# NVIDIA/makani

Hardware: NVIDIA H100
Metric: SFNO-block fwd+bwd samples/sec (higher is better)
Workload: dtype tf32

## Files before the change

makani_b200/csrc/dft.cu:

```cuda
#include "umma_common.cuh"
#include "dft_math.cuh"
#include <cmath>
#include <cstdlib>
#include <vector>

namespace b200sht {

int umma_available();

constexpr int kDftMaxHalf = 95;
constexpr int kDftSynWorkers = 10;
constexpr int kDftSynThreads = 32 * (kDftSynWorkers + 2);
constexpr int kDftSynStages = 4;
__host__ __device__ constexpr int dft_out_box(int N2) {
  int d = N2 < 32 ? N2 : 32;
  while (N2 % d != 0) --d;
  return 8 * d;
}

struct DftTables {
  float* et;
  float* eb;
  float2* tw;
  float* zeros;
  int N2, half, M2, nkb;
};

bool dft_shape_ok(int nlon, int mmax) {
  if (nlon % 8 != 0) return false;
  const int N2 = nlon / 8;
  return N2 >= 2 && N2 / 2 <= kDftMaxHalf && (mmax + 7) / 8 <= 32 && mmax <= nlon / 2 + 1;
}

__global__ void dft_tables_kernel(float* et, float* eb, float2* tw, int N2, int half, int M2, int nkb, int nlon) {
  const int i = blockIdx.x * blockDim.x + threadIdx.x;
  if (i < 2 * 128 * 32) {
    const int m2 = i % 32, row = i / 32, p = (row >> 3) & 1, j2 = 8 * (row >> 4) + (row & 7);
    float v = 0.f;
    if (j2 <= half && m2 < M2) {
      const long long t = ((long long)m2 * j2) % N2;
      const double ang = 2.0 * M_PI * (double)t / (double)N2;
      v = tf32_rn((float)(p == 0 ? cos(ang) : sin(ang)));
    }
    et[i] = v;
  }
  if (i < nkb * 2 * 32 * 32) {
    const int jl = i % 32, m2 = (i / 32) % 32, p = (i / 1024) % 2, kb = i / 2048;
    const int j2 = kb * 32 + jl;
    float v = 0.f;
    if (j2 <= half && m2 < M2) {
      const long long t = ((long long)m2 * j2) % N2;
      const double ang = 2.0 * M_PI * (double)t / (double)N2;
      v = tf32_rn((float)(p == 0 ? cos(ang) : sin(ang)));
      if (2 * j2 == N2) v *= 0.5f;
    }
    eb[i] = v;
  }
  if (i < 8 * N2) {
    const int j2 = i % N2, c = i / N2;
    const double ang = 2.0 * M_PI * (double)(c * j2) / (double)nlon;
    tw[i] = make_float2((float)cos(ang), (float)sin(ang));
  }
}

int dft_plan_init(Plan* pl) {
  pl->dft_state = nullptr;
  if (!umma_available()) return -1;
  if (!dft_shape_ok(pl->nlon, pl->mmax)) return -1;
  DftTables* t = new DftTables();
  t->N2 = pl->nlon / 8; t->half = t->N2 / 2; t->M2 = (pl->mmax + 7) / 8;
  t->nkb = (t->half + 1 + 31) / 32;
  t->et = nullptr; t->eb = nullptr; t->tw = nullptr; t->zeros = nullptr;
  const size_t neb = (size_t)t->nkb * 2 * 32 * 32;
  cudaError_t e = cudaMalloc(&t->et, sizeof(float) * 2 * 128 * 32);
  if (e == cudaSuccess) e = cudaMalloc(&t->eb, sizeof(float) * neb);
  if (e == cudaSuccess) e = cudaMalloc(&t->tw, sizeof(float2) * 8 * t->N2);
  if (e == cudaSuccess) e = cudaMalloc(&t->zeros, sizeof(float) * 8 * t->N2);
  if (e == cudaSuccess) e = cudaMemset(t->zeros, 0, sizeof(float) * 8 * t->N2);
  if (e == cudaSuccess) {
    const int n = 8192 > 8 * t->N2 ? 8192 : 8 * t->N2;
    dft_tables_kernel<<<(n + 255) / 256, 256>>>(t->et, t->eb, t->tw, t->N2, t->half, t->M2, t->nkb, pl->nlon);
    e = cudaGetLastError();
    if (e == cudaSuccess) e = cudaStreamSynchronize(0);
  }
  if (e != cudaSuccess) {
    cudaFree(t->et); cudaFree(t->eb); cudaFree(t->tw); cudaFree(t->zeros);
    delete t;
    return -1;
  }
  pl->dft_state = t;
  return 0;
}

void dft_plan_destroy(Plan* pl) {
  DftTables* t = static_cast<DftTables*>(pl->dft_state);
  if (!t) return;
  cudaFree(t->et); cudaFree(t->eb); cudaFree(t->tw); cudaFree(t->zeros);
  delete t;
  pl->dft_state = nullptr;
}

static bool dft_enabled() {
  static const int on = [] { const char* e = getenv("B200SHT_DFT"); return e ? atoi(e) : 1; }();
  return on != 0;
}
bool dft_usable(const Plan* pl) { return pl->dft_state != nullptr && dft_enabled(); }

static unsigned long long* g_dft_prof = nullptr;
static unsigned long long* dft_prof_buffer() {
  static const int on = [] { const char* e = getenv("B200SHT_DFT_PROF"); return e ? atoi(e) : 0; }();
  if (!on) return nullptr;
  if (!g_dft_prof) {
    if (cudaMalloc(&g_dft_prof, 16 * sizeof(unsigned long long)) != cudaSuccess) { g_dft_prof = nullptr; return nullptr; }
    cudaMemset(g_dft_prof, 0, 16 * sizeof(unsigned long long));
  }
  return g_dft_prof;
}
int dft_profile_read(unsigned long long* out16) {
  if (!g_dft_prof) { for (int i = 0; i < 16; ++i) out16[i] = 0; return 0; }
  B200_CHECK_CUDA(cudaDeviceSynchronize());
  B200_CHECK_CUDA(cudaMemcpy(out16, g_dft_prof, 16 * sizeof(unsigned long long), cudaMemcpyDeviceToHost));
  B200_CHECK_CUDA(cudaMemset(g_dft_prof, 0, 16 * sizeof(unsigned long long)));
  return 0;
}
#ifdef B200SHT_DFT_PROFILE
constexpr bool kDftProfile = true;
#else
constexpr bool kDftProfile = false;
#endif
__device__ __forceinline__ void prof_wait(unsigned long long* prof, int slot, uint64_t* bar, uint32_t parity, bool lead) {
  if (!kDftProfile || prof == nullptr) { mbar_wait(bar, parity); return; }
  const long long t0 = clock64();
  mbar_wait(bar, parity);
  if (lead) atomicAdd(prof + slot, (unsigned long long)(clock64() - t0));
}

static int make_tmap_out(CUtensorMap* tm, void* base, bool bf16, int nlon, int nlat, long long rows, int ow) {
  TmapKey key;
  memset(&key, 0, sizeof(key));
  key.base = base; key.rank = 3; key.kind = bf16 ? 7 : 6;
  key.dims[0] = nlon; key.dims[1] = nlat; key.dims[2] = rows; key.box[0] = ow;
  int slot = 0;
  if (tmap_lookup(key, tm, &slot)) return 0;
  PFN_encodeTiled enc = get_encode();
  if (!enc) { set_error("cuTensorMapEncodeTiled is unavailable"); return B200SHT_ERR_UNSUPPORTED; }
  static thread_local bool ctx_bound = false;
  if (!ctx_bound) { cudaFree(nullptr); ctx_bound = true; }
  const int es = bf16 ? 2 : 4;
  cuuint64_t gd[3] = {(cuuint64_t)nlon, (cuuint64_t)nlat, (cuuint64_t)rows};
  cuuint64_t gst[2] = {(cuuint64_t)nlon * es, (cuuint64_t)nlon * nlat * es};
  cuuint32_t bx[3] = {(cuuint32_t)ow, 8, 1}, el[3] = {1, 1, 1};
  if (gst[0] % 16 != 0 || (reinterpret_cast<uintptr_t>(base) & 15) != 0 || (ow * es) % 16 != 0) {
    set_error("tensor map (output): base / row pitch / box row not 16-byte aligned");
    return B200SHT_ERR_INVALID;
  }
  CUresult r = enc(tm, bf16 ? CU_TENSOR_MAP_DATA_TYPE_BFLOAT16 : CU_TENSOR_MAP_DATA_TYPE_FLOAT32, 3, base, gd, gst, bx, el,
                   CU_TENSOR_MAP_INTERLEAVE_NONE, CU_TENSOR_MAP_SWIZZLE_NONE, CU_TENSOR_MAP_L2_PROMOTION_L2_256B, CU_TENSOR_MAP_FLOAT_OOB_FILL_NONE);
  if (r != CUDA_SUCCESS) { set_error("cuTensorMapEncodeTiled (output) failed (%d)", (int)r); return B200SHT_ERR_CUDA; }
  tmap_store(key, tm, slot);
  return 0;
}

template <typename T> __device__ __forceinline__ void st_out(T* p, float v);
template <> __device__ __forceinline__ void st_out<float>(float* p, float v) { *p = v; }
template <> __device__ __forceinline__ void st_out<__nv_bfloat16>(__nv_bfloat16* p, float v) { *p = __float2bfloat16_rn(v); }
template <typename T> __device__ __forceinline__ uint32_t ld_raw(const T* p);
template <> __device__ __forceinline__ uint32_t ld_raw<float>(const float* p) { return __float_as_uint(__ldg(p)); }
template <> __device__ __forceinline__ uint32_t ld_raw<__nv_bfloat16>(const __nv_bfloat16* p) { return (uint32_t)__ldg(reinterpret_cast<const unsigned short*>(p)); }

#ifndef B200_DFT_TF32_MODE
#define B200_DFT_TF32_MODE 2
#endif
constexpr float kTruncComp = 1.0f + 0.0009765625f / 3.0f;
__device__ __forceinline__ float tf32_operand(float v) {
#if B200_DFT_TF32_MODE == 0
  return tf32_rn(v);
#elif B200_DFT_TF32_MODE == 1
  return __uint_as_float((__float_as_uint(v) + 0x1000u) & 0xffffe000u);
#else
  return v;
#endif
}
__device__ __forceinline__ float tf32_operand_unscaled(float v) {
#if B200_DFT_TF32_MODE == 2
  return v * kTruncComp;
#else
  return tf32_operand(v);
#endif
}

__device__ __forceinline__ pr pr_operand(pr v) { return make_pr(tf32_operand(v.v.x), tf32_operand(v.v.y)); }
__device__ __forceinline__ pr pr_operand_unscaled(pr v) {
#if B200_DFT_TF32_MODE == 2
  return rmul(v, kTruncComp);
#else
  return pr_operand(v);
#endif
}

template <typename T> __device__ __forceinline__ float ld_in(const T* p);
template <> __device__ __forceinline__ float ld_in<float>(const float* p) { return __ldg(p); }
template <> __device__ __forceinline__ float ld_in<__nv_bfloat16>(const __nv_bfloat16* p) {
  return __uint_as_float((uint32_t)__ldg(reinterpret_cast<const unsigned short*>(p)) << 16);
}

struct DftSynParams {
  alignas(64) CUtensorMap tmZ;
  alignas(64) CUtensorMap tmE;
  alignas(64) CUtensorMap tmY;
  const float* Z;
  const float2* tw;
  const float* rowscale;
  const float* bias;
  unsigned long long* prof;
  int R, C, nlat, nlon, kp, mmax, N2, half, M2, mode, ntiles, ktiles, has_nyq, ow;
  int kt0, kt_all;
};

template <typename T>
__global__ void __launch_bounds__(kDftSynThreads, 1) dft_synthesis_kernel(const __grid_constant__ DftSynParams p) {
  extern __shared__ uint8_t smem_raw[];
  __shared__ unsigned long long prof_s[16];
  unsigned long long* const prof = (kDftProfile && p.prof) ? prof_s : nullptr;
  if (kDftProfile && threadIdx.x < 16) prof_s[threadIdx.x] = 0;
  const uint32_t raw = smem_u32(smem_raw);
  const uint32_t base = (raw + 1023u) & ~1023u;
  uint8_t* gbase = smem_raw + (base - raw);
  const int N2 = p.N2;
  const int nlon = 8 * N2;
  const int ow = p.ow;
  const uint32_t obytes = (8u * nlon * sizeof(T) + 1023u) & ~1023u;
  const uint32_t sA = base, sB = base + 32768, sO = sB + kDftSynStages * 16384;
  T* const outS = reinterpret_cast<T*>(gbase + (sO - base));
  float2* tws = reinterpret_cast<float2*>(gbase + (sO - base) + 2 * obytes);
  uint64_t* bars = reinterpret_cast<uint64_t*>(reinterpret_cast<uint8_t*>(tws) + ((8 * N2 * 8 + 15) & ~15));
  uint64_t* full = bars;
  uint64_t* empty = full + kDftSynStages;
  uint64_t* e_full = empty + kDftSynStages;
  uint64_t* staged = e_full + 1;
  uint64_t* ofree = staged + 2;

  const int warp = __shfl_sync(0xffffffffu, (int)(threadIdx.x >> 5), 0), lane = threadIdx.x & 31;
  pdl_trigger();
  const int nblk = (p.half + 8) / 8;
  const int nwork = kDftSynWorkers < 2 * nblk ? kDftSynWorkers : 2 * nblk;
  const bool is_tma = (warp == kDftSynWorkers), is_store = (warp == kDftSynWorkers + 1);

  if (threadIdx.x == 0) {
    for (int s = 0; s < kDftSynStages; ++s) { mbar_init(&full[s], 1); mbar_init(&empty[s], nblk); }
    mbar_init(e_full, 1);
    for (int b = 0; b < 2; ++b) { mbar_init(&staged[b], 32 * nblk); mbar_init(&ofree[b], 1); }
    fence_barrier_init();
    prefetch_tmap(&p.tmZ);
    prefetch_tmap(&p.tmE);
    prefetch_tmap(&p.tmY);
  }
  for (int i = threadIdx.x; i < 8 * p.N2; i += blockDim.x) tws[i] = p.tw[i];
  __syncthreads();
  const long long t_cta0 = (kDftProfile && p.prof && threadIdx.x == 0) ? clock64() : 0;
  pdl_wait();

  if (is_tma) {
    if (lane == 0) {
      mbar_expect_tx(e_full, 32768);
      tma_load_2d(sA, &p.tmE, e_full, 0, 0);
      tma_load_2d(sA + 16384, &p.tmE, e_full, 0, 128);
      int n = 0;
      for (int ti = blockIdx.x; ti < p.ntiles; ti += gridDim.x, ++n) {
        const int s = n % kDftSynStages, it = n / kDftSynStages;
        if (it > 0) prof_wait(prof, 8, &empty[s], (it - 1) & 1, true);
        mbar_expect_tx(&full[s], 16384);
        const uint32_t st = sB + s * 16384;
        const int ta = (ti / p.ktiles) * p.kt_all + p.kt0 + ti % p.ktiles;
        tma_load_5d(st, &p.tmZ, &full[s], 0, 0, 0, 0, ta);
        tma_load_5d(st + 4096, &p.tmZ, &full[s], 0, 1, 0, 0, ta);
        tma_load_5d(st + 8192, &p.tmZ, &full[s], 0, 0, 0, 1, ta);
        tma_load_5d(st + 12288, &p.tmZ, &full[s], 0, 1, 0, 1, ta);
      }
    }
    __syncwarp();
  } else if (is_store) {
    if (lane == 0) {
      int n = 0;
      for (int ti = blockIdx.x; ti < p.ntiles; ti += gridDim.x, ++n) {
        const int b = n & 1;
        prof_wait(prof, 11, &staged[b], (n >> 1) & 1, true);
        const int r = ti / p.ktiles, k0 = (p.kt0 + ti - r * p.ktiles) * 8;
// ... 112 lines not shown
      }
    }
  }
  __syncthreads();
  if (kDftProfile && p.prof && threadIdx.x == 0) prof_s[12] = (unsigned long long)(clock64() - t_cta0);
  if (kDftProfile) __syncthreads();
  if (kDftProfile && p.prof && threadIdx.x < 16) atomicAdd(p.prof + threadIdx.x, prof_s[threadIdx.x]);
}

int dft_synthesis(const Plan* pl, const float* Z, void* y, int dtype, int B, int C, const float* bias, int mode, cudaStream_t st, int k_begin, int k_end) {
  const DftTables* t = static_cast<const DftTables*>(pl->dft_state);
  B200_REQUIRE(t != nullptr, "dft_synthesis: plan has no DFT tables");
  const int R = B * C;
  DftSynParams p;
  memset(&p, 0, sizeof(p));
  p.Z = Z; p.tw = t->tw; p.rowscale = pl->d_rowscale; p.bias = bias; p.prof = dft_prof_buffer();
  p.R = R; p.C = C; p.nlat = pl->nlat; p.nlon = pl->nlon; p.kp = pl->kp; p.mmax = pl->mmax;
  p.N2 = t->N2; p.half = t->half; p.mode = mode;
  if (k_end < 0 || k_end > pl->kp) k_end = pl->kp;
  B200_REQUIRE(k_begin >= 0 && k_begin % 8 == 0 && k_begin < k_end, "dft_synthesis: bad latitude range [%d, %d)", k_begin, k_end);
  p.kt_all = pl->kp / 8; p.kt0 = k_begin / 8;
  p.ktiles = (k_end - k_begin + 7) / 8; p.ntiles = R * p.ktiles;
  p.has_nyq = (pl->mmax == pl->nlon / 2 + 1) ? 1 : 0;
  p.M2 = t->M2;
  {
    long long d[5] = {32, 2, t->M2, 2, (long long)R * (pl->kp / 8)}, s[5] = {1, 32, 64, (long long)t->M2 * 64, 2ll * t->M2 * 64};
    int bx[5] = {32, 1, 32, 1, 1};
    int rc = make_tmap(&p.tmZ, Z, 5, d, s, bx);
    if (rc) return rc;
  }
  {
    long long d[2] = {32, 256}, s[2] = {1, 32};
    int bx[2] = {32, 128};
    int rc = make_tmap(&p.tmE, t->et, 2, d, s, bx);
    if (rc) return rc;
  }
  const bool bf16 = (dtype == B200SHT_BF16);
  p.ow = dft_out_box(t->N2);
  {
    int rc = make_tmap_out(&p.tmY, y, bf16, pl->nlon, pl->nlat, R, p.ow);
    if (rc) return rc;
  }
  const size_t obytes = (8 * (size_t)pl->nlon * (bf16 ? 2 : 4) + 1023) & ~(size_t)1023;
  const size_t smem = 1024 + 32768 + (size_t)kDftSynStages * 16384 + 2 * obytes + ((8 * (size_t)t->N2 * 8 + 15) & ~(size_t)15) +
                      (2 * kDftSynStages + 5) * 8;
  const int sms = usable_sms(pl->sm_count > 0 ? pl->sm_count : 132);
  const int ctas = p.ntiles < sms ? p.ntiles : sms;
#define B200_LAUNCH_SYN(TT)                                                                                          \
  do {                                                                                                                \
    struct Tag {};                                                                                                    \
    B200_CHECK_CUDA((ensure_dynamic_smem<Tag>(dft_synthesis_kernel<TT>, smem)));                                     \
    B200_CHECK_CUDA(launch_pdl(dft_synthesis_kernel<TT>, dim3(ctas), dim3(kDftSynThreads), smem, st, p));            \
  } while (0)
  if (bf16) { B200_LAUNCH_SYN(__nv_bfloat16); } else { B200_LAUNCH_SYN(float); }
#undef B200_LAUNCH_SYN
  B200_CHECK_LAUNCH();
  return 0;
}

__host__ __device__ constexpr int dft_box_group(int N2, int es) { return (N2 * es) % 16 == 0 ? 1 : (2 * N2 * es) % 16 == 0 ? 2 : (4 * N2 * es) % 16 == 0 ? 4 : 8; }

static int make_tmap_segments(CUtensorMap* tm, const void* base, bool bf16, int nlon, int gs, long long rows, int box_cols) {
  TmapKey key;
  memset(&key, 0, sizeof(key));
  key.base = base; key.rank = 3; key.kind = bf16 ? 5 : 4;
  key.dims[0] = nlon; key.dims[1] = gs; key.dims[2] = rows; key.box[0] = box_cols;
  int slot = 0;
  if (tmap_lookup(key, tm, &slot)) return 0;
  PFN_encodeTiled enc = get_encode();
  if (!enc) { set_error("cuTensorMapEncodeTiled is unavailable"); return B200SHT_ERR_UNSUPPORTED; }
  static thread_local bool ctx_bound = false;
  if (!ctx_bound) { cudaFree(nullptr); ctx_bound = true; }
  const int es = bf16 ? 2 : 4, N2 = nlon / 8;
  cuuint64_t gd[3] = {(cuuint64_t)gs * N2, (cuuint64_t)(8 / gs), (cuuint64_t)rows};
  cuuint64_t gst[2] = {(cuuint64_t)gs * N2 * es, (cuuint64_t)nlon * es};
  cuuint32_t bx[3] = {(cuuint32_t)box_cols, (cuuint32_t)(8 / gs), 16}, el[3] = {1, 1, 1};
  if (gst[0] % 16 != 0 || gst[1] % 16 != 0 || (reinterpret_cast<uintptr_t>(base) & 15) != 0 || (box_cols * es) % 16 != 0) {
    set_error("tensor map (segments): base / pitch / box row not 16-byte aligned");
    return B200SHT_ERR_INVALID;
  }
  CUresult r = enc(tm, bf16 ? CU_TENSOR_MAP_DATA_TYPE_BFLOAT16 : CU_TENSOR_MAP_DATA_TYPE_FLOAT32, 3, const_cast<void*>(base), gd, gst, bx, el,
                   CU_TENSOR_MAP_INTERLEAVE_NONE, CU_TENSOR_MAP_SWIZZLE_NONE, CU_TENSOR_MAP_L2_PROMOTION_L2_256B, CU_TENSOR_MAP_FLOAT_OOB_FILL_NONE);
  if (r != CUDA_SUCCESS) { set_error("cuTensorMapEncodeTiled (segments) failed (%d)", (int)r); return B200SHT_ERR_CUDA; }
  tmap_store(key, tm, slot);
  return 0;
}

constexpr int kDftAnaStages = 2;
constexpr int kDftAnaMma = 8, kDftAnaLoader = 8, kDftAnaProd0 = 9, kDftAnaThreads = 512;

struct DftAnaParams {
  alignas(64) CUtensorMap tmB;
  alignas(64) CUtensorMap tmXc;
  alignas(64) CUtensorMap tmXp;
  float* X;
  const float2* tw;
  const float* rowscale;
  unsigned long long* prof;
  int R, nlat, nlon, kp, mmax, N2, half, M2, nkb, mode, round_tf32, ntiles, ktiles, nraw, gs;
  int kt0;
};

template <typename T, int N2T>
__global__ void __launch_bounds__(kDftAnaThreads, 1) dft_analysis_kernel(const __grid_constant__ DftAnaParams p) {
  extern __shared__ uint8_t smem_raw[];
  __shared__ unsigned long long prof_s[16];
  unsigned long long* const prof = (kDftProfile && p.prof) ? prof_s : nullptr;
  if (kDftProfile && threadIdx.x < 16) prof_s[threadIdx.x] = 0;
  const uint32_t raw = smem_u32(smem_raw);
  const uint32_t base = (raw + 1023u) & ~1023u;
  uint8_t* gbase = smem_raw + (base - raw);
  constexpr int kAl = 16 / (int)sizeof(T);
  constexpr int kWc = (sizeof(T) == 2) ? 40 : 32, kWp = (sizeof(T) == 2) ? 40 : 36;
  constexpr uint32_t kColBytes = 16u * kWc * sizeof(T), kParBytes = 16u * kWp * sizeof(T);
  constexpr uint32_t kRawBytes = 8u * (kColBytes + kParBytes);
  const uint32_t oB = 0, oA = 3 * 8192, oR = oA + kDftAnaStages * 65536, oT = oR + (uint32_t)p.nraw * kRawBytes, oBar = oT + 3 * 7 * 32 * 8;
  const uint32_t sBm = base + oB, sAr = base + oA, sRaw = base + oR;
  uint8_t* gA = gbase + oA;
  const uint8_t* gR = gbase + oR;
  float2* twS = reinterpret_cast<float2*>(gbase + oT);
  uint64_t* full = reinterpret_cast<uint64_t*>(gbase + oBar);
  uint64_t* empty = full + kDftAnaStages;
  uint64_t* raw_full = empty + kDftAnaStages;
  uint64_t* raw_empty = raw_full + 4;
  uint64_t* b_full = raw_empty + 4;

  const int warp = __shfl_sync(0xffffffffu, (int)(threadIdx.x >> 5), 0), lane = threadIdx.x & 31;
  pdl_trigger();
  const int nkb = p.nkb;
  const int N2 = N2T > 0 ? N2T : p.N2;
  const int gs = N2T > 0 ? dft_box_group(N2T, (int)sizeof(T)) : p.gs;
  for (int i = threadIdx.x; i < nkb * 7 * 32; i += blockDim.x) {
    const int ln = i & 31, c = (i >> 5) % 7 + 1, kb = i / 224;
    const int j2 = 32 * kb + ln;
    float2 w = (j2 <= p.half) ? p.tw[c * N2 + j2] : make_float2(1.f, 0.f);
#if B200_DFT_TF32_MODE == 2
    w.x *= kTruncComp; w.y *= kTruncComp;
#endif
    twS[i] = w;
  }
  if (threadIdx.x == 0) {
    for (int s = 0; s < kDftAnaStages; ++s) { mbar_init(&full[s], 8); mbar_init(&empty[s], kDftAnaMma); }
    for (int s = 0; s < p.nraw; ++s) { mbar_init(&raw_full[s], 1); mbar_init(&raw_empty[s], 8); }
    mbar_init(b_full, 1);
    fence_barrier_init();
    prefetch_tmap(&p.tmB);
    prefetch_tmap(&p.tmXc);
    prefetch_tmap(&p.tmXp);
  }
  for (int i = threadIdx.x; i < kDftAnaStages * 2 * 512; i += blockDim.x) {
    const int st = i >> 10, pl = (i >> 9) & 1, off = i & 511;
    reinterpret_cast<float*>(gA + (size_t)st * 65536)[(pl ? 12288 : 4096) + off] = 0.f;
  }
  __syncthreads();
  const long long t_cta0 = (kDftProfile && p.prof && threadIdx.x == 0) ? clock64() : 0;
  pdl_wait();

  if (warp == kDftAnaLoader) {
    if (lane == 0) {
      mbar_expect_tx(b_full, (uint32_t)nkb * 8192);
      for (int kb = 0; kb < nkb; ++kb) {
        tma_load_2d(sBm + kb * 8192, &p.tmB, b_full, 0, kb * 64);
        tma_load_2d(sBm + kb * 8192 + 4096, &p.tmB, b_full, 0, kb * 64 + 32);
      }
      int n = 0;
      for (int ti = blockIdx.x; ti < p.ntiles; ti += gridDim.x, ++n) {
        const int r = ti / p.ktiles, row0 = r * p.nlat + (p.kt0 + ti - r * p.ktiles) * 16;
        for (int kb = 0; kb < nkb; ++kb) {
          const int g = n * nkb + kb, rs = g % p.nraw, it = g / p.nraw;
          if (it > 0) prof_wait(prof, 2, &raw_empty[rs], (it - 1) & 1, true);
          mbar_expect_tx(&raw_full[rs], kRawBytes);
          const uint32_t dst = sRaw + rs * kRawBytes;
#pragma unroll
          for (int gm = 0; gm < 8; ++gm) {
            if (gm >= gs) break;
            const int sc = N2 * gm + 32 * kb, sp = N2 * gm + N2 - 32 * kb - 31;
            tma_load_3d(dst + gm * (8 / gs) * kColBytes, &p.tmXc, &raw_full[rs], (sc / kAl) * kAl, 0, row0);
            tma_load_3d(dst + 8 * kColBytes + gm * (8 / gs) * kParBytes, &p.tmXp, &raw_full[rs], sp < 0 ? 0 : (sp / kAl) * kAl, 0, row0);
          }
        }
      }
    }
    __syncwarp();
  } else if (warp < kDftAnaMma) {
    const size_t plane = (size_t)p.R * p.kp;
    const float tcomp = p.round_tf32 ? kTruncComp : 1.f;
    const uint32_t tmask = p.round_tf32 ? 0xffffe000u : 0xffffffffu;
    const int c = warp, gq = lane >> 2, q = lane & 3;
    mbar_wait(b_full, 0);
    int n = 0;
    for (int ti = blockIdx.x; ti < p.ntiles; ti += gridDim.x, ++n) {
      const int r = ti / p.ktiles, k0 = (p.kt0 + ti - r * p.ktiles) * 16;
      float xr[4][4], xi[4][4];
#pragma unroll
      for (int j = 0; j < 4; ++j)
#pragma unroll
        for (int e = 0; e < 4; ++e) { xr[j][e] = 0.f; xi[j][e] = 0.f; }
      for (int kb = 0; kb < nkb; ++kb) {
        const int g = n * nkb + kb, s = g % kDftAnaStages, it = g / kDftAnaStages;
        prof_wait(prof, 3, &full[s], it & 1, lane == 0);
        const uint8_t* const a0 = gA + (size_t)s * 65536;
        const uint8_t* const bc = gbase + oB + kb * 8192;
#pragma unroll
        for (int half = 0; half < 2; ++half) {
          const uint32_t col = 32 * q + 16 * half;
          uint4 av[4][2];
#pragma unroll
          for (int pl = 0; pl < 4; ++pl)
#pragma unroll
            for (int h = 0; h < 2; ++h) av[pl][h] = lds128(a0 + pl * 16384, (16 * c + gq + 8 * h) * 128 + col);
#pragma unroll
          for (int cs = 0; cs < 2; ++cs) {
            uint4 bv[4];
#pragma unroll
            for (int j = 0; j < 4; ++j) bv[j] = lds128(bc + cs * 4096, (8 * j + gq) * 128 + col);
            const int pr_ = cs ? 3 : 0, pi_ = cs ? 2 : 1;
#pragma unroll
            for (int t = 0; t < 2; ++t) {
              uint32_t far_[4], fai[4];
              far_[0] = t ? av[pr_][0].z : av[pr_][0].x; far_[1] = t ? av[pr_][1].z : av[pr_][1].x;
              far_[2] = t ? av[pr_][0].w : av[pr_][0].y; far_[3] = t ? av[pr_][1].w : av[pr_][1].y;
              fai[0] = t ? av[pi_][0].z : av[pi_][0].x; fai[1] = t ? av[pi_][1].z : av[pi_][1].x;
              fai[2] = t ? av[pi_][0].w : av[pi_][0].y; fai[3] = t ? av[pi_][1].w : av[pi_][1].y;
              if (cs) frag_neg(fai, fai);
#pragma unroll
              for (int j = 0; j < 4; ++j) {
                const uint32_t fb[2] = {t ? bv[j].z : bv[j].x, t ? bv[j].w : bv[j].y};
                mma_tf32(xr[j], far_, fb);
                mma_tf32(xi[j], fai, fb);
              }
            }
          }
        }
        __syncwarp();
        if (lane == 0) mbar_arrive(&empty[s]);
      }
      if (prof && lane == 0) atomicAdd(prof + 5, 1ull);
#pragma unroll
      for (int h = 0; h < 2; ++h) {
        const int k = k0 + gq + 8 * h;
        if (k >= p.kp) continue;
        const float rs = (p.mode == 0) ? ((k < p.nlat) ? __ldg(p.rowscale + k) : 0.f) : 1.f;
        float* xb = p.X + (size_t)r * p.kp + k;
#pragma unroll
        for (int j = 0; j < 4; ++j)
#pragma unroll
          for (int e = 0; e < 2; ++e) {
            const int m = c + 8 * (8 * j + 2 * q + e);
            if (m >= p.mmax) continue;
            const float sc = ((p.mode == 0) ? rs : ((m == 0 || 2 * m == p.nlon) ? 1.f : 2.f)) * tcomp;
            float* dst = xb + (size_t)m * 2 * plane;
            dst[0] = __uint_as_float(__float_as_uint(xr[j][2 * h + e] * sc) & tmask);
            dst[plane] = __uint_as_float(__float_as_uint(xi[j][2 * h + e] * sc) & tmask);
          }
      }
    }
  } else {
    const int pw = warp - kDftAnaProd0;
    constexpr int nprod = kDftAnaThreads / 32 - kDftAnaProd0;
    static_assert(nprod >= 1 && nprod <= 8, "every producer warp must take an item of every K-block (8 items each)");
    constexpr bool kBf16 = (sizeof(T) == 2);
    const T* const rawS = reinterpret_cast<const T*>(gR);
    int n = 0;
    for (int ti = blockIdx.x; ti < p.ntiles; ti += gridDim.x, ++n) {
      const int r = ti / p.ktiles, kt16 = (p.kt0 + ti - r * p.ktiles) * 16;
      for (int item = pw; item < 8 * nkb; item += nprod) {
        const int kb = item >> 3, q = item & 7;
        const int k0 = kt16 + 2 * q;
        const int g = n * nkb + kb;
        const int j2 = 32 * kb + lane;
        const int rs = g % p.nraw;
        prof_wait(prof, 0, &raw_full[rs], (g / p.nraw) & 1, lane == 0);
        if (prof && lane == 0) atomicAdd(prof + 7, 1ull);
        const T* const rb = rawS + (size_t)rs * (kRawBytes / sizeof(T));
        pr xa[8], xb[8];
#pragma unroll
        for (int j1 = 0; j1 < 8; ++j1) {
          const int gm = j1 % gs, ga = j1 / gs, npb = 8 / gs;
          const int sc = N2 * gm + 32 * kb, sp = N2 * gm + N2 - 32 * kb - 31;
          const int ic = sc - (sc / kAl) * kAl + lane;
          int ip = N2 * gm + N2 - j2 - (sp < 0 ? 0 : (sp / kAl) * kAl);
          ip = ip < 0 ? 0 : (ip > kWp - 1 ? kWp - 1 : ip);
          const T* b0 = rb + gm * (16 * npb * kWc) + (2 * q) * (npb * kWc) + ga * kWc;
          const T* b1 = rb + 8 * (16 * kWc) + gm * (16 * npb * kWp) + (2 * q) * (npb * kWp) + ga * kWp;
          const int rowc = npb * kWc, rowp = npb * kWp;
          if constexpr (kBf16) {
            xa[j1] = make_pr(__uint_as_float((uint32_t)reinterpret_cast<const unsigned short*>(b0)[ic] << 16),
                             __uint_as_float((uint32_t)reinterpret_cast<const unsigned short*>(b0)[rowc + ic] << 16));
            xb[j1] = make_pr(__uint_as_float((uint32_t)reinterpret_cast<const unsigned short*>(b1)[ip] << 16),
                             __uint_as_float((uint32_t)reinterpret_cast<const unsigned short*>(b1)[rowp + ip] << 16));
          } else {
            xa[j1] = make_pr(reinterpret_cast<const float*>(b0)[ic], reinterpret_cast<const float*>(b0)[rowc + ic]);
            xb[j1] = make_pr(reinterpret_cast<const float*>(b1)[ip], reinterpret_cast<const float*>(b1)[rowp + ip]);
          }
        }
        __syncwarp();
        if (lane == 0) mbar_arrive(&raw_empty[rs]);
        if (kb == 0) {
#pragma unroll
          for (int j1 = 0; j1 < 8; ++j1) xb[j1] = (lane == 0) ? make_pr(0.f, 0.f) : xb[j1];
        }
        if (k0 + 1 >= p.nlat) {
          const bool row0ok = k0 < p.nlat;
#pragma unroll
          for (int j1 = 0; j1 < 8; ++j1) {
            xa[j1] = make_pr(row0ok ? xa[j1].v.x : 0.f, 0.f);
            xb[j1] = make_pr(row0ok ? xb[j1].v.x : 0.f, 0.f);
          }
        }
        pr er[8], ei[8], br[8], bi[8];
        float2 tw[8], tp[8];
        tw[0] = make_float2(1.f, 0.f);
        const float2* const twl = twS + kb * 224 + lane;
#pragma unroll
        for (int c = 1; c < 8; ++c) tw[c] = twl[(c - 1) * 32];
        dft_partner_twiddles(tw, tp);
        dft_ana_radix8<pr>(xa, tw, er, ei);
        dft_ana_radix8<pr>(xb, tp, br, bi);
        const int s = g % kDftAnaStages, it = g / kDftAnaStages;
        if (it > 0) prof_wait(prof, 1, &empty[s], (it - 1) & 1, lane == 0);
        float* const stg = reinterpret_cast<float*>(gA + (size_t)s * 65536);
        const int kr0 = 2 * q;
        float* const d0 = stg + kr0 * 32 + ((((lane >> 2) ^ (kr0 & 7)) << 2) | (lane & 3));
        float* const d1 = stg + (kr0 + 1) * 32 + ((((lane >> 2) ^ ((kr0 + 1) & 7)) << 2) | (lane & 3));
#pragma unroll
        for (int c = 0; c < 8; ++c) {
          pr ye_r = er[c] + br[c], yo_r = er[c] - br[c];
          if (c == 0) { ye_r = pr_operand_unscaled(ye_r); yo_r = pr_operand_unscaled(yo_r); }
          else { ye_r = pr_operand(ye_r); yo_r = pr_operand(yo_r); }
          d0[c * 512] = ye_r.v.x; d1[c * 512] = ye_r.v.y;
          d0[8192 + c * 512] = yo_r.v.x; d1[8192 + c * 512] = yo_r.v.y;
          if (c != 0) {
            const pr ye_i = pr_operand(ei[c] + bi[c]), yo_i = pr_operand(ei[c] - bi[c]);
            d0[4096 + c * 512] = ye_i.v.x; d1[4096 + c * 512] = ye_i.v.y;
            d0[12288 + c * 512] = yo_i.v.x; d1[12288 + c * 512] = yo_i.v.y;
          }
        }
        fence_proxy_async();
        __syncwarp();
        if (lane == 0) mbar_arrive(&full[s]);
      }
    }
  }
  __syncthreads();
  if (kDftProfile && p.prof && threadIdx.x == 0) prof_s[6] = (unsigned long long)(clock64() - t_cta0);
  if (kDftProfile) __syncthreads();
  if (kDftProfile && p.prof && threadIdx.x < 16) atomicAdd(p.prof + threadIdx.x, prof_s[threadIdx.x]);
}

int dft_analysis(const Plan* pl, const void* x, int dtype, int B, int C, float* X, int mode, int round_tf32, cudaStream_t st, int k_begin, int k_end) {
  const DftTables* t = static_cast<const DftTables*>(pl->dft_state);
  B200_REQUIRE(t != nullptr, "dft_analysis: plan has no DFT tables");
  const int R = B * C;
  DftAnaParams p;
  memset(&p, 0, sizeof(p));
  p.X = X; p.tw = t->tw; p.rowscale = pl->d_rowscale; p.prof = dft_prof_buffer();
  p.R = R; p.nlat = pl->nlat; p.nlon = pl->nlon; p.kp = pl->kp; p.mmax = pl->mmax;
  p.N2 = t->N2; p.half = t->half; p.M2 = t->M2; p.nkb = t->nkb; p.mode = mode; p.round_tf32 = round_tf32;
  if (k_end < 0 || k_end > pl->kp) k_end = pl->kp;
  B200_REQUIRE(k_begin >= 0 && k_begin % 16 == 0 && k_begin < k_end, "dft_analysis: bad latitude range [%d, %d)", k_begin, k_end);
  p.kt0 = k_begin / 16;
  p.ktiles = (k_end - k_begin + 15) / 16; p.ntiles = R * p.ktiles;
  const bool bf16 = (dtype == B200SHT_BF16);
  p.nraw = bf16 ? 3 : 2;
  {
    long long d[2] = {32, (long long)t->nkb * 64}, s[2] = {1, 32};
    int bx[2] = {32, 32};
    int rc = make_tmap(&p.tmB, t->eb, 2, d, s, bx);
    if (rc) return rc;
  }
  B200_REQUIRE(bf16 || t->N2 % 4 == 0, "dft_analysis: fp32 input needs nlon %% 32 == 0 (16-byte aligned TMA boxes)");
  {
    p.gs = dft_box_group(t->N2, bf16 ? 2 : 4);
    int rc = make_tmap_segments(&p.tmXc, x, bf16, pl->nlon, p.gs, (long long)R * pl->nlat, bf16 ? 40 : 32);
    if (!rc) rc = make_tmap_segments(&p.tmXp, x, bf16, pl->nlon, p.gs, (long long)R * pl->nlat, bf16 ? 40 : 36);
    if (rc) return rc;
  }
  const size_t raw_bytes = bf16 ? (size_t)8 * 16 * (40 + 40) * 2 : (size_t)8 * 16 * (32 + 36) * 4;
  const size_t smem = 1024 + 3 * 8192 + (size_t)kDftAnaStages * 65536 + p.nraw * raw_bytes + 3 * 7 * 32 * 8 + 256;
  const int sms = usable_sms(pl->sm_count > 0 ? pl->sm_count : 132);
  const int ctas = p.ntiles < sms ? p.ntiles : sms;
  const int threads = kDftAnaThreads;
#define B200_LAUNCH_ANA(TT, NN)                                                                                                          \
  do {                                                                                                                                  \
    struct Tag {};                                                                                                                        \
    B200_CHECK_CUDA((ensure_dynamic_smem<Tag>(dft_analysis_kernel<TT, NN>, smem)));                                                      \
    B200_CHECK_CUDA(launch_pdl(dft_analysis_kernel<TT, NN>, dim3(ctas), dim3(threads), smem, st, p));                                                                         \
  } while (0)
#define B200_DISPATCH_ANA(TT)                                            \
  switch (t->N2) {                                                       \
    case 180: B200_LAUNCH_ANA(TT, 180); break;            \
    case 90: B200_LAUNCH_ANA(TT, 90); break;              \
    case 60: B200_LAUNCH_ANA(TT, 60); break;              \
    default: B200_LAUNCH_ANA(TT, 0); break;                              \
  }
  if (bf16) { B200_DISPATCH_ANA(__nv_bfloat16) } else { B200_DISPATCH_ANA(float) }
#undef B200_DISPATCH_ANA
#undef B200_LAUNCH_ANA
  B200_CHECK_LAUNCH();
  return 0;
}

int dft_host(int N, int mmax, int direction, int mode, const float* rowscale, const float* in, float* out) {
  if (!dft_shape_ok(N, mmax)) { set_error("debug_dft_host: unsupported (nlon=%d, mmax=%d)", N, mmax); return B200SHT_ERR_UNSUPPORTED; }
  const int N2 = N / 8, half = N2 / 2, M2 = (mmax + 7) / 8;
  const float rs = rowscale ? rowscale[0] : 1.f;
  auto twid = [&](int j, float2* tw) {
    for (int c = 0; c < 8; ++c) {
      const double a = 2.0 * M_PI * (double)(c * j) / (double)N;
      tw[c] = make_float2((float)cos(a), (float)sin(a));
    }
  };
  if (direction == 1) {
    std::vector<double> zr(8 * M2, 0.0), zi(8 * M2, 0.0);
    for (int m = 0; m < mmax; ++m) { zr[m] = in[2 * m]; zi[m] = in[2 * m + 1]; }
    const bool has_nyq = (mmax == N / 2 + 1);
    for (int j2 = 0; j2 <= half; ++j2) {
      float s1[8], s2[8], s3[8], s4[8];
      for (int c = 0; c < 8; ++c) {
        double a1 = 0, a2 = 0, a3 = 0, a4 = 0;
        for (int m2 = 0; m2 < M2; ++m2) {
          const double b = 2.0 * M_PI * (double)(((long long)m2 * j2) % N2) / (double)N2;
          a1 += cos(b) * zr[c + 8 * m2]; a2 += sin(b) * zi[c + 8 * m2]; a3 += sin(b) * zr[c + 8 * m2]; a4 += cos(b) * zi[c + 8 * m2];
        }
        s1[c] = (float)a1; s2[c] = (float)a2; s3[c] = (float)a3; s4[c] = (float)a4;
      }
      float2 tw[8], tp[8];
      twid(j2, tw);
      dft_partner_twiddles(tw, tp);
      for (int side = 0; side < 2; ++side) {
        if (side == 1 && (j2 == 0 || 2 * j2 == N2)) continue;
        const int jj = side ? N2 - j2 : j2;
        float vr[8], vi[8], x[8];
        for (int c = 0; c < 8; ++c) {
          vr[c] = side ? s1[c] + s2[c] : s1[c] - s2[c];
          vi[c] = side ? s4[c] - s3[c] : s3[c] + s4[c];
        }
        dft_syn_radix8<float>(vr, vi, side ? tp : tw, x);
        for (int j1 = 0; j1 < 8; ++j1) {
          const int j = N2 * j1 + jj;
          float v = x[j1];
          if (mode == 0) {
            v = 2.f * v - (float)zr[0];
            if (has_nyq) v -= (float)zr[N / 2] * ((j & 1) ? -1.f : 1.f);
          } else {
            v *= rs;
          }
          out[j] = v;
        }
      }
    }
    return 0;
  }
  std::vector<double> dre(8 * M2, 0.0), dim(8 * M2, 0.0);
  for (int j2 = 0; j2 <= half; ++j2) {
    float2 tw[8], tp[8];
    twid(j2, tw);
    dft_partner_twiddles(tw, tp);
    float xa[8], er[8], ei[8], orr[8], oi[8];
    for (int j1 = 0; j1 < 8; ++j1) xa[j1] = in[N2 * j1 + j2];
    dft_ana_radix8<float>(xa, tw, er, ei);
    const bool paired = (j2 != 0 && 2 * j2 != N2);
    if (paired) {
      float xb[8], br[8], bi[8];
      for (int j1 = 0; j1 < 8; ++j1) xb[j1] = in[N2 * j1 + N2 - j2];
      dft_ana_radix8<float>(xb, tp, br, bi);
      for (int c = 0; c < 8; ++c) { orr[c] = er[c] - br[c]; oi[c] = ei[c] - bi[c]; er[c] += br[c]; ei[c] += bi[c]; }
    } else {
      for (int c = 0; c < 8; ++c) { orr[c] = 0.f; oi[c] = 0.f; }
    }
    for (int c = 0; c < 8; ++c)
      for (int m2 = 0; m2 < M2; ++m2) {
        const double b = 2.0 * M_PI * (double)(((long long)m2 * j2) % N2) / (double)N2;
// ... 14 lines not shown
```

makani_b200/csrc/umma_common.cuh:

```cuda
#pragma once
#include "common.cuh"
#include <cuda.h>
#include <mutex>
#include <cstring>

namespace b200sht {

__device__ __forceinline__ uint32_t smem_u32(const void* p) { return (uint32_t)__cvta_generic_to_shared(p); }

__device__ __forceinline__ void mbar_init(uint64_t* bar, uint32_t count) {
  asm volatile("mbarrier.init.shared::cta.b64 [%0], %1;" ::"r"(smem_u32(bar)), "r"(count) : "memory");
}
__device__ __forceinline__ void fence_barrier_init() { asm volatile("fence.mbarrier_init.release.cluster;" ::: "memory"); }
__device__ __forceinline__ void mbar_expect_tx(uint64_t* bar, uint32_t bytes) {
  asm volatile("mbarrier.arrive.expect_tx.shared::cta.b64 _, [%0], %1;" ::"r"(smem_u32(bar)), "r"(bytes) : "memory");
}
__device__ __forceinline__ uint32_t mbar_try_wait(uint64_t* bar, uint32_t parity) {
  uint32_t done;
  asm volatile(
      "{\n\t.reg .pred p;\n\t"
      "mbarrier.try_wait.parity.shared::cta.b64 p, [%1], %2;\n\t"
      "selp.u32 %0, 1, 0, p;\n\t}"
      : "=r"(done)
      : "r"(smem_u32(bar)), "r"(parity)
      : "memory");
  return done;
}
__device__ __forceinline__ uint32_t mbar_try_wait_hint(uint64_t* bar, uint32_t parity, uint32_t ns) {
  uint32_t done;
  asm volatile(
      "{\n\t.reg .pred p;\n\t"
      "mbarrier.try_wait.parity.shared::cta.b64 p, [%1], %2, %3;\n\t"
      "selp.u32 %0, 1, 0, p;\n\t}"
      : "=r"(done)
      : "r"(smem_u32(bar)), "r"(parity), "r"(ns)
      : "memory");
  return done;
}
__device__ __forceinline__ void mbar_wait(uint64_t* bar, uint32_t parity) {
  if (mbar_try_wait(bar, parity)) return;
  uint32_t spins = 0;
  long long t0 = 0;
  while (!mbar_try_wait_hint(bar, parity, 20000u)) {
    if ((++spins & 255u) == 0) {
      const long long t = clock64();
      if (t0 == 0) t0 = t;
      else if (t - t0 > 4000000000LL) {
        printf("b200sht: mbarrier timeout block (%d,%d,%d) thread %d\n", blockIdx.x, blockIdx.y, blockIdx.z, threadIdx.x);
        __trap();
      }
    }
  }
}

__device__ __forceinline__ void mbar_wait_nocall(uint64_t* bar, uint32_t parity) {
  if (mbar_try_wait(bar, parity)) return;
  uint32_t spins = 0;
  long long t0 = 0;
  while (!mbar_try_wait_hint(bar, parity, 20000u)) {
    if ((++spins & 255u) == 0) {
      const long long t = clock64();
      if (t0 == 0) t0 = t;
      else if (t - t0 > 4000000000LL) __trap();
    }
  }
}

__device__ __forceinline__ void mbar_wait_relaxed(uint64_t* bar, uint32_t parity, uint32_t ns) {
  if (mbar_try_wait(bar, parity)) return;
  uint32_t spins = 0;
  long long t0 = 0;
  for (;;) {
    __nanosleep(ns);
    if (mbar_try_wait(bar, parity)) return;
    if ((++spins & 255u) == 0) {
      const long long t = clock64();
      if (t0 == 0) t0 = t;
      else if (t - t0 > 4000000000LL) {
        printf("b200sht: mbarrier timeout block (%d,%d,%d) thread %d\n", blockIdx.x, blockIdx.y, blockIdx.z, threadIdx.x);
        __trap();
      }
    }
  }
}

__device__ __forceinline__ void tma_load_3d(uint32_t dst, const CUtensorMap* tm, uint64_t* bar, int c0, int c1, int c2) {
  asm volatile("cp.async.bulk.tensor.3d.shared::cluster.global.tile.mbarrier::complete_tx::bytes [%0], [%1, {%3, %4, %5}], [%2];" ::"r"(dst),
               "l"(tm), "r"(smem_u32(bar)), "r"(c0), "r"(c1), "r"(c2)
               : "memory");
}
__device__ __forceinline__ void tma_load_4d(uint32_t dst, const CUtensorMap* tm, uint64_t* bar, int c0, int c1, int c2, int c3) {
  asm volatile("cp.async.bulk.tensor.4d.shared::cluster.global.tile.mbarrier::complete_tx::bytes [%0], [%1, {%3, %4, %5, %6}], [%2];" ::"r"(dst),
               "l"(tm), "r"(smem_u32(bar)), "r"(c0), "r"(c1), "r"(c2), "r"(c3)
               : "memory");
}
__device__ __forceinline__ void tma_load_5d(uint32_t dst, const CUtensorMap* tm, uint64_t* bar, int c0, int c1, int c2, int c3, int c4) {
  asm volatile("cp.async.bulk.tensor.5d.shared::cluster.global.tile.mbarrier::complete_tx::bytes [%0], [%1, {%3, %4, %5, %6, %7}], [%2];" ::"r"(dst),
               "l"(tm), "r"(smem_u32(bar)), "r"(c0), "r"(c1), "r"(c2), "r"(c3), "r"(c4)
               : "memory");
}
__device__ __forceinline__ void prefetch_tmap(const CUtensorMap* tm) { asm volatile("prefetch.tensormap [%0];" ::"l"(tm) : "memory"); }

__device__ __forceinline__ uint32_t swz128(uint32_t off) { return off ^ ((off >> 3) & 0x70u); }
template <bool MN>
__device__ __forceinline__ uint32_t ld_op(const uint8_t* tile, int r, int k) {
  const uint32_t off = MN ? (uint32_t)((r >> 5) * 4096 + k * 128 + (r & 31) * 4) : (uint32_t)(r * 128 + k * 4);
  return *reinterpret_cast<const uint32_t*>(tile + swz128(off));
}
__device__ __forceinline__ uint2 lds64(const uint8_t* tile, uint32_t off) { return *reinterpret_cast<const uint2*>(tile + swz128(off)); }
__device__ __forceinline__ uint4 lds128(const uint8_t* tile, uint32_t off) { return *reinterpret_cast<const uint4*>(tile + swz128(off)); }
template <bool MN>
__device__ __forceinline__ void frag_a(const uint8_t* tile, int r0, int k0, uint32_t (&a)[4]) {
  const int lane = threadIdx.x & 31, g = lane >> 2, q = lane & 3;
  a[0] = ld_op<MN>(tile, r0 + g, k0 + q);
  a[1] = ld_op<MN>(tile, r0 + g + 8, k0 + q);
  a[2] = ld_op<MN>(tile, r0 + g, k0 + q + 4);
  a[3] = ld_op<MN>(tile, r0 + g + 8, k0 + q + 4);
}
template <bool MN>
__device__ __forceinline__ void frag_b(const uint8_t* tile, int n0, int k0, uint32_t (&b)[2]) {
  const int lane = threadIdx.x & 31, g = lane >> 2, q = lane & 3;
  b[0] = ld_op<MN>(tile, n0 + g, k0 + q);
  b[1] = ld_op<MN>(tile, n0 + g, k0 + q + 4);
}
__device__ __forceinline__ void frag_neg(const uint32_t (&a)[4], uint32_t (&n)[4]) {
#pragma unroll
  for (int i = 0; i < 4; ++i) n[i] = a[i] ^ 0x80000000u;
}
__device__ __forceinline__ void mma_tf32(float (&d)[4], const uint32_t (&a)[4], const uint32_t (&b)[2]) {
  asm volatile("mma.sync.aligned.m16n8k8.row.col.f32.tf32.tf32.f32 {%0, %1, %2, %3}, {%4, %5, %6, %7}, {%8, %9}, {%0, %1, %2, %3};"
               : "+f"(d[0]), "+f"(d[1]), "+f"(d[2]), "+f"(d[3])
               : "r"(a[0]), "r"(a[1]), "r"(a[2]), "r"(a[3]), "r"(b[0]), "r"(b[1]));
}

__device__ __forceinline__ uint64_t wgmma_desc_kmajor(uint32_t saddr) {
  return (uint64_t)((saddr & 0x3FFFFu) >> 4) | (1ull << 16) | ((uint64_t)(1024 >> 4) << 32) | (1ull << 62);
}
__device__ __forceinline__ void wgmma_fence() { asm volatile("wgmma.fence.sync.aligned;" ::: "memory"); }
__device__ __forceinline__ void wgmma_commit() { asm volatile("wgmma.commit_group.sync.aligned;" ::: "memory"); }
template <int N>
__device__ __forceinline__ void wgmma_wait() { asm volatile("wgmma.wait_group.sync.aligned %0;" ::"n"(N) : "memory"); }
template <int NA>
__device__ __forceinline__ void wgmma_fence_operands(float (&d)[NA][4]) {
#pragma unroll
  for (int j = 0; j < NA; ++j)
#pragma unroll
    for (int e = 0; e < 4; ++e) asm volatile("" : "+f"(d[j][e])::"memory");
}

__device__ __forceinline__ void mbar_arrive(uint64_t* bar) {
  asm volatile("mbarrier.arrive.shared::cta.b64 _, [%0];" ::"r"(smem_u32(bar)) : "memory");
}
__device__ __forceinline__ void tma_load_2d(uint32_t dst, const CUtensorMap* tm, uint64_t* bar, int c0, int c1) {
  asm volatile("cp.async.bulk.tensor.2d.shared::cluster.global.tile.mbarrier::complete_tx::bytes [%0], [%1, {%3, %4}], [%2];" ::"r"(dst),
               "l"(tm), "r"(smem_u32(bar)), "r"(c0), "r"(c1)
               : "memory");
}
__device__ __forceinline__ void fence_proxy_async() { asm volatile("fence.proxy.async.shared::cta;" ::: "memory"); }

__device__ __forceinline__ void tma_store_3d(const CUtensorMap* tm, uint32_t src, int c0, int c1, int c2) {
  asm volatile("cp.async.bulk.tensor.3d.global.shared::cta.bulk_group [%0, {%2, %3, %4}], [%1];" ::"l"(tm), "r"(src), "r"(c0), "r"(c1), "r"(c2)
               : "memory");
}
__device__ __forceinline__ void tma_store_5d(const CUtensorMap* tm, uint32_t src, int c0, int c1, int c2, int c3, int c4) {
  asm volatile("cp.async.bulk.tensor.5d.global.shared::cta.bulk_group [%0, {%2, %3, %4, %5, %6}], [%1];" ::"l"(tm), "r"(src), "r"(c0), "r"(c1),
               "r"(c2), "r"(c3), "r"(c4)
               : "memory");
}
__device__ __forceinline__ void bulk_commit() { asm volatile("cp.async.bulk.commit_group;" ::: "memory"); }
template <int N>
__device__ __forceinline__ void bulk_wait_read() { asm volatile("cp.async.bulk.wait_group.read %0;" ::"n"(N) : "memory"); }
__device__ __forceinline__ void bulk_wait_read0() { bulk_wait_read<0>(); }
__device__ __forceinline__ void bulk_wait0() { asm volatile("cp.async.bulk.wait_group 0;" ::: "memory"); }

typedef CUresult (*PFN_encodeTiled)(CUtensorMap*, CUtensorMapDataType, cuuint32_t, void*, const cuuint64_t*, const cuuint64_t*, const cuuint32_t*,
                                    const cuuint32_t*, CUtensorMapInterleave, CUtensorMapSwizzle, CUtensorMapL2promotion, CUtensorMapFloatOOBfill);

inline PFN_encodeTiled get_encode() {
  static PFN_encodeTiled fn = nullptr;
  static std::once_flag once;
  std::call_once(once, [] {
    void* ptr = nullptr;
    cudaDriverEntryPointQueryResult q;
    if (cudaGetDriverEntryPoint("cuTensorMapEncodeTiled", &ptr, cudaEnableDefault, &q) == cudaSuccess && q == cudaDriverEntryPointSuccess)
      fn = reinterpret_cast<PFN_encodeTiled>(ptr);
  });
  return fn;
}

struct TmapKey {
  const void* base;
  long long dims[5], strides[5];
  int box[5];
  int rank, kind;
};
struct TmapCache {
  static constexpr int kSlots = 128;
  CUtensorMap maps[kSlots];
  TmapKey keys[kSlots];
  bool used[kSlots];
};
inline TmapCache& tmap_cache() {
  static thread_local TmapCache* c = [] { TmapCache* p = new TmapCache(); memset(p->used, 0, sizeof(p->used)); return p; }();
  return *c;
}
inline int tmap_slot(const TmapKey& k) {
  const unsigned char* b = reinterpret_cast<const unsigned char*>(&k);
  uint64_t h = 1469598103934665603ull;
  for (size_t i = 0; i < sizeof(TmapKey); ++i) { h ^= b[i]; h *= 1099511628211ull; }
  return (int)(h % TmapCache::kSlots);
}
inline bool tmap_lookup(const TmapKey& k, CUtensorMap* tm, int* slot) {
  TmapCache& c = tmap_cache();
  *slot = tmap_slot(k);
  if (c.used[*slot] && memcmp(&c.keys[*slot], &k, sizeof(TmapKey)) == 0) { memcpy(tm, &c.maps[*slot], sizeof(CUtensorMap)); return true; }
  return false;
}
inline void tmap_store(const TmapKey& k, const CUtensorMap* tm, int slot) {
  TmapCache& c = tmap_cache();
  memcpy(&c.maps[slot], tm, sizeof(CUtensorMap));
  c.keys[slot] = k;
  c.used[slot] = true;
}

inline int make_tmap(CUtensorMap* tm, const void* base, int rank, const long long* dims, const long long* strides, const int* box,
                     bool swizzle = true) {
  TmapKey key;
  memset(&key, 0, sizeof(key));
  key.base = base; key.rank = rank; key.kind = swizzle ? 0 : 1;
  for (int i = 0; i < rank; ++i) { key.dims[i] = dims[i]; key.strides[i] = i ? strides[i] : 1; key.box[i] = box[i]; }
  int slot = 0;
  if (tmap_lookup(key, tm, &slot)) return 0;
  PFN_encodeTiled enc = get_encode();
  if (!enc) { set_error("cuTensorMapEncodeTiled is unavailable"); return B200SHT_ERR_UNSUPPORTED; }
  static thread_local bool ctx_bound = false;
  if (!ctx_bound) { cudaFree(nullptr); ctx_bound = true; }
  cuuint64_t gd[5], gs[4];
  cuuint32_t bx[5], es[5];
  for (int i = 0; i < rank; ++i) { gd[i] = (cuuint64_t)dims[i]; bx[i] = (cuuint32_t)box[i]; es[i] = 1; }
  for (int i = 1; i < rank; ++i) {
    gs[i - 1] = (cuuint64_t)strides[i] * 4;
    if (gs[i - 1] % 16 != 0) { set_error("tensor map stride %lld floats is not 16-byte aligned", strides[i]); return B200SHT_ERR_INVALID; }
  }
  if ((reinterpret_cast<uintptr_t>(base) & 15) != 0) { set_error("tensor map base is not 16-byte aligned"); return B200SHT_ERR_INVALID; }
  CUresult r = enc(tm, CU_TENSOR_MAP_DATA_TYPE_FLOAT32, (cuuint32_t)rank, const_cast<void*>(base), gd, gs, bx, es, CU_TENSOR_MAP_INTERLEAVE_NONE,
                   swizzle ? CU_TENSOR_MAP_SWIZZLE_128B : CU_TENSOR_MAP_SWIZZLE_NONE, CU_TENSOR_MAP_L2_PROMOTION_L2_256B,
                   CU_TENSOR_MAP_FLOAT_OOB_FILL_NONE);
  if (r != CUDA_SUCCESS) { set_error("cuTensorMapEncodeTiled failed (%d), rank %d", (int)r, rank); return B200SHT_ERR_CUDA; }
  tmap_store(key, tm, slot);
  return 0;
}


inline int make_tmap_rows(CUtensorMap* tm, const void* base, bool bf16, long long cols, long long rows, int box_cols, int box_rows) {
  PFN_encodeTiled enc = get_encode();
  if (!enc) { set_error("cuTensorMapEncodeTiled is unavailable"); return B200SHT_ERR_UNSUPPORTED; }
  static thread_local bool ctx_bound = false;
  if (!ctx_bound) { cudaFree(nullptr); ctx_bound = true; }
  const int es = bf16 ? 2 : 4;
  cuuint64_t gd[2] = {(cuuint64_t)cols, (cuuint64_t)rows}, gs[1] = {(cuuint64_t)cols * es};
  cuuint32_t bx[2] = {(cuuint32_t)box_cols, (cuuint32_t)box_rows}, el[2] = {1, 1};
  if (gs[0] % 16 != 0 || (reinterpret_cast<uintptr_t>(base) & 15) != 0 || (box_cols * es) % 16 != 0) {
    set_error("tensor map (rows): base / row pitch / box row not 16-byte aligned");
    return B200SHT_ERR_INVALID;
  }
  CUresult r = enc(tm, bf16 ? CU_TENSOR_MAP_DATA_TYPE_BFLOAT16 : CU_TENSOR_MAP_DATA_TYPE_FLOAT32, 2, const_cast<void*>(base), gd, gs, bx, el,
                   CU_TENSOR_MAP_INTERLEAVE_NONE, CU_TENSOR_MAP_SWIZZLE_NONE, CU_TENSOR_MAP_L2_PROMOTION_L2_256B, CU_TENSOR_MAP_FLOAT_OOB_FILL_NONE);
  if (r != CUDA_SUCCESS) { set_error("cuTensorMapEncodeTiled (rows) failed (%d)", (int)r); return B200SHT_ERR_CUDA; }
  return 0;
}

}
```

Baseline: 748.5.

## Replace mma.sync fragment loop in DFT analysis with warpgroup wgmma TF32

The MMA warps of the DFT analysis kernel now issue asynchronous warpgroup wgmma TF32 instructions from shared-memory descriptors, instead of loading swizzled fragments into registers and issuing many mma.sync m16n8k8 ops. Real and imaginary results go into one accumulator array, and the sign flip for the imaginary parts moves into the wgmma scale arguments. Barrier waits switch to a non-call mbar_wait variant, and proxy fences are added so generic-proxy stores become visible to the async proxy. The aim is to cut shared-memory fragment loads and register pressure, at the cost of a commit/wait per k-block that serialises the MMA with the stage release.

After: 764.7, median of 6. 2.2% higher.

```diff
diff --git a/makani_b200/csrc/dft.cu b/makani_b200/csrc/dft.cu
--- a/makani_b200/csrc/dft.cu
+++ b/makani_b200/csrc/dft.cu
@@ -1,4 +1,5 @@
 #include "umma_common.cuh"
+#include "wgmma_tf32.cuh"
 #include "dft_math.cuh"
 #include <cmath>
 #include <cstdlib>
@@ -128,11 +129,12 @@
 #else
 constexpr bool kDftProfile = false;
 #endif
+template <bool kNoCall = false>
 __device__ __forceinline__ void prof_wait(unsigned long long* prof, int slot, uint64_t* bar, uint32_t parity, bool lead) {
-  if (!kDftProfile || prof == nullptr) { mbar_wait(bar, parity); return; }
-  const long long t0 = clock64();
-  mbar_wait(bar, parity);
-  if (lead) atomicAdd(prof + slot, (unsigned long long)(clock64() - t0));
+  const long long t0 = (kDftProfile && prof != nullptr) ? clock64() : 0;
+  if constexpr (kNoCall) mbar_wait_nocall(bar, parity);
+  else mbar_wait(bar, parity);
+  if (kDftProfile && prof != nullptr && lead) atomicAdd(prof + slot, (unsigned long long)(clock64() - t0));
 }
 
 static int make_tmap_out(CUtensorMap* tm, void* base, bool bf16, int nlon, int nlat, long long rows, int ow) {
@@ -551,6 +553,7 @@
     const int st = i >> 10, pl = (i >> 9) & 1, off = i & 511;
     reinterpret_cast<float*>(gA + (size_t)st * 65536)[(pl ? 12288 : 4096) + off] = 0.f;
   }
+  fence_proxy_async();
   __syncthreads();
   const long long t_cta0 = (kDftProfile && p.prof && threadIdx.x == 0) ? clock64() : 0;
   pdl_wait();
@@ -567,7 +570,7 @@
         const int r = ti / p.ktiles, row0 = r * p.nlat + (p.kt0 + ti - r * p.ktiles) * 16;
         for (int kb = 0; kb < nkb; ++kb) {
           const int g = n * nkb + kb, rs = g % p.nraw, it = g / p.nraw;
-          if (it > 0) prof_wait(prof, 2, &raw_empty[rs], (it - 1) & 1, true);
+          if (it > 0) prof_wait<true>(prof, 2, &raw_empty[rs], (it - 1) & 1, true);
           mbar_expect_tx(&raw_full[rs], kRawBytes);
           const uint32_t dst = sRaw + rs * kRawBytes;
 #pragma unroll
@@ -585,55 +588,33 @@
     const size_t plane = (size_t)p.R * p.kp;
     const float tcomp = p.round_tf32 ? kTruncComp : 1.f;
     const uint32_t tmask = p.round_tf32 ? 0xffffe000u : 0xffffffffu;
-    const int c = warp, gq = lane >> 2, q = lane & 3;
-    mbar_wait(b_full, 0);
+    const int c = warp, gq = lane >> 2, q = lane & 3, wg = warp >> 2;
+    mbar_wait_nocall(b_full, 0);
     int n = 0;
     for (int ti = blockIdx.x; ti < p.ntiles; ti += gridDim.x, ++n) {
       const int r = ti / p.ktiles, k0 = (p.kt0 + ti - r * p.ktiles) * 16;
-      float xr[4][4], xi[4][4];
-#pragma unroll
-      for (int j = 0; j < 4; ++j)
-#pragma unroll
-        for (int e = 0; e < 4; ++e) { xr[j][e] = 0.f; xi[j][e] = 0.f; }
+      float acc[8][4];
       for (int kb = 0; kb < nkb; ++kb) {
         const int g = n * nkb + kb, s = g % kDftAnaStages, it = g / kDftAnaStages;
-        prof_wait(prof, 3, &full[s], it & 1, lane == 0);
-        const uint8_t* const a0 = gA + (size_t)s * 65536;
-        const uint8_t* const bc = gbase + oB + kb * 8192;
-#pragma unroll
-        for (int half = 0; half < 2; ++half) {
-          const uint32_t col = 32 * q + 16 * half;
-          uint4 av[4][2];
-#pragma unroll
-          for (int pl = 0; pl < 4; ++pl)
-#pragma unroll
-            for (int h = 0; h < 2; ++h) av[pl][h] = lds128(a0 + pl * 16384, (16 * c + gq + 8 * h) * 128 + col);
-#pragma unroll
-          for (int cs = 0; cs < 2; ++cs) {
-            uint4 bv[4];
-#pragma unroll
-            for (int j = 0; j < 4; ++j) bv[j] = lds128(bc + cs * 4096, (8 * j + gq) * 128 + col);
-            const int pr_ = cs ? 3 : 0, pi_ = cs ? 2 : 1;
-#pragma unroll
-            for (int t = 0; t < 2; ++t) {
-              uint32_t far_[4], fai[4];
-              far_[0] = t ? av[pr_][0].z : av[pr_][0].x; far_[1] = t ? av[pr_][1].z : av[pr_][1].x;
-              far_[2] = t ? av[pr_][0].w : av[pr_][0].y; far_[3] = t ? av[pr_][1].w : av[pr_][1].y;
-              fai[0] = t ? av[pi_][0].z : av[pi_][0].x; fai[1] = t ? av[pi_][1].z : av[pi_][1].x;
-              fai[2] = t ? av[pi_][0].w : av[pi_][0].y; fai[3] = t ? av[pi_][1].w : av[pi_][1].y;
-              if (cs) frag_neg(fai, fai);
-#pragma unroll
-              for (int j = 0; j < 4; ++j) {
-                const uint32_t fb[2] = {t ? bv[j].z : bv[j].x, t ? bv[j].w : bv[j].y};
-                mma_tf32(xr[j], far_, fb);
-                mma_tf32(xi[j], fai, fb);
-              }
-            }
-          }
-        }
-        __syncwarp();
+        prof_wait<true>(prof, 3, &full[s], it & 1, lane == 0);
+        const uint32_t st = sAr + s * 65536 + 8192 * wg;
+        const uint64_t ye_r = wgmma_desc_kmajor(st), ye_i = wgmma_desc_kmajor(st + 16384);
+        const uint64_t yo_r = wgmma_desc_kmajor(st + 32768), yo_i = wgmma_desc_kmajor(st + 49152);
+        const uint64_t ec = wgmma_desc_kmajor(sBm + kb * 8192), es = wgmma_desc_kmajor(sBm + kb * 8192 + 4096);
+        wgmma_fence();
+#pragma unroll
+        for (int k = 0; k < 4; ++k) {
+          const int sd = (k > 0 || kb > 0) ? 1 : 0;
+          wgmma_tf32<32, 1, 8, 0>(acc, ye_r + 2 * k, ec + 2 * k, sd);
+          wgmma_tf32<32, 1, 8, 4>(acc, ye_i + 2 * k, ec + 2 * k, sd);
+          wgmma_tf32<32, 1, 8, 0>(acc, yo_i + 2 * k, es + 2 * k, 1);
+          wgmma_tf32<32, -1, 8, 4>(acc, yo_r + 2 * k, es + 2 * k, 1);
+        }
+        wgmma_commit();
+        wgmma_wait<0>();
         if (lane == 0) mbar_arrive(&empty[s]);
       }
+      wgmma_fence_operands(acc);
       if (prof && lane == 0) atomicAdd(prof + 5, 1ull);
 #pragma unroll
       for (int h = 0; h < 2; ++h) {
@@ -649,8 +630,8 @@
             if (m >= p.mmax) continue;
             const float sc = ((p.mode == 0) ? rs : ((m == 0 || 2 * m == p.nlon) ? 1.f : 2.f)) * tcomp;
             float* dst = xb + (size_t)m * 2 * plane;
-            dst[0] = __uint_as_float(__float_as_uint(xr[j][2 * h + e] * sc) & tmask);
-            dst[plane] = __uint_as_float(__float_as_uint(xi[j][2 * h + e] * sc) & tmask);
+            dst[0] = __uint_as_float(__float_as_uint(acc[j][2 * h + e] * sc) & tmask);
+            dst[plane] = __uint_as_float(__float_as_uint(acc[4 + j][2 * h + e] * sc) & tmask);
           }
       }
     }
@@ -669,7 +650,7 @@
         const int g = n * nkb + kb;
         const int j2 = 32 * kb + lane;
         const int rs = g % p.nraw;
-        prof_wait(prof, 0, &raw_full[rs], (g / p.nraw) & 1, lane == 0);
+        prof_wait<true>(prof, 0, &raw_full[rs], (g / p.nraw) & 1, lane == 0);
         if (prof && lane == 0) atomicAdd(prof + 7, 1ull);
         const T* const rb = rawS + (size_t)rs * (kRawBytes / sizeof(T));
         pr xa[8], xb[8];
@@ -693,6 +674,7 @@
             xb[j1] = make_pr(reinterpret_cast<const float*>(b1)[ip], reinterpret_cast<const float*>(b1)[rowp + ip]);
           }
         }
+        __threadfence_block();
         __syncwarp();
         if (lane == 0) mbar_arrive(&raw_empty[rs]);
         if (kb == 0) {
@@ -717,7 +699,7 @@
         dft_ana_radix8<pr>(xa, tw, er, ei);
         dft_ana_radix8<pr>(xb, tp, br, bi);
         const int s = g % kDftAnaStages, it = g / kDftAnaStages;
-        if (it > 0) prof_wait(prof, 1, &empty[s], (it - 1) & 1, lane == 0);
+        if (it > 0) prof_wait<true>(prof, 1, &empty[s], (it - 1) & 1, lane == 0);
         float* const stg = reinterpret_cast<float*>(gA + (size_t)s * 65536);
         const int kr0 = 2 * q;
         float* const d0 = stg + kr0 * 32 + ((((lane >> 2) ^ (kr0 & 7)) << 2) | (lane & 3));
diff --git a/makani_b200/csrc/umma_common.cuh b/makani_b200/csrc/umma_common.cuh
--- a/makani_b200/csrc/umma_common.cuh
+++ b/makani_b200/csrc/umma_common.cuh
@@ -122,10 +122,6 @@
   const int lane = threadIdx.x & 31, g = lane >> 2, q = lane & 3;
   b[0] = ld_op<MN>(tile, n0 + g, k0 + q);
   b[1] = ld_op<MN>(tile, n0 + g, k0 + q + 4);
-}
-__device__ __forceinline__ void frag_neg(const uint32_t (&a)[4], uint32_t (&n)[4]) {
-#pragma unroll
-  for (int i = 0; i < 4; ++i) n[i] = a[i] ^ 0x80000000u;
 }
 __device__ __forceinline__ void mma_tf32(float (&d)[4], const uint32_t (&a)[4], const uint32_t (&b)[2]) {
   asm volatile("mma.sync.aligned.m16n8k8.row.col.f32.tf32.tf32.f32 {%0, %1, %2, %3}, {%4, %5, %6, %7}, {%8, %9}, {%0, %1, %2, %3};"
```
